# vinits5/bullet-envs

Hardware: AMD Instinct MI355X
Metric: env-steps/sec (whole node), 16-link snake, 4096 envs/GPU (higher is better)
Workload: dtype f32

## Files before the change

bullet-envs_amd/csrc/snk_dynamics.hpp:

```cpp
#pragma once
#include "snk_lds.hpp"
#include "snk_model.hpp"
#include "snk_wave.hpp"

namespace snk {

#ifndef SNK_SCALAR_DYNAMICS
__device__ __forceinline__ float quad_yzx(float x) {
    return __int_as_float(__builtin_amdgcn_update_dpp(0, __float_as_int(x), 0xC9, 0xf, 0xf, true));
}
__device__ __forceinline__ float quad_zxy(float x) {
    return __int_as_float(__builtin_amdgcn_update_dpp(0, __float_as_int(x), 0xD2, 0xf, 0xf, true));
}
__device__ __forceinline__ float lane_cross(float a_yzx, float a_zxy, float b) {
#pragma clang fp contract(off)
    return __builtin_fmaf(a_yzx, quad_zxy(b), -(a_zxy * quad_yzx(b)));
}
struct LaneVel {
    float w, v, za, zl;
};
__device__ __forceinline__ LaneVel lane_vel_step(float wp, float vp, float ax, float rb, float qdb) {
#pragma clang fp contract(off)
    const float wy = quad_yzx(wp), wz = quad_zxy(wp);
    const float cr = lane_cross(wy, wz, rb);
    LaneVel o;
    o.w = __builtin_fmaf(ax, qdb, wp);
    o.v = vp + cr;
    o.za = lane_cross(wy, wz, ax) * qdb;
    o.zl = lane_cross(wy, wz, cr);
    return o;
}
#endif

template <class LT>
__device__ void fk_vel(LT& L, const DevModel& M, int lane) {
    constexpr int N = LT::kN;
    const float* bs = L.base();
    float Rp[9];
    quat_rot(bs[3], bs[4], bs[5], bs[6], Rp);
    f3 op = ld3(bs), wp = ld3(bs + 7), vp = ld3(bs + 10);
    if (lane == 0) {
#pragma unroll
        for (int i = 0; i < 9; i++) L.R[0][i] = Rp[i];
        st3(L.o[0], op); st3(L.w[0], wp); st3(L.v[0], vp);
        st3(L.r[0], mk3(0, 0, 0)); st3(L.ax[0], mk3(0, 0, 0));
#pragma unroll
        for (int i = 0; i < 6; i++) L.zeta[0][i] = 0.f;
    }
    float snv = 0.f, csv = 1.f;
    if (lane < N) sincosf(L.q()[lane], &snv, &csv);
#ifndef SNK_SCALAR_DYNAMICS
    const int ln = launder_lane(lane);
    const int c = ln & 3, cc = c < 3 ? c : 2;
    float C0 = c == 0 ? Rp[0] : (c == 1 ? Rp[3] : Rp[6]);
    float C1 = c == 0 ? Rp[1] : (c == 1 ? Rp[4] : Rp[7]);
    float C2 = c == 0 ? Rp[2] : (c == 1 ? Rp[5] : Rp[8]);
    float opv = bs[cc], wpv = bs[7 + cc], vpv = bs[10 + cc];
#pragma unroll 4
    for (int b = 1; b <= N; b++) {
#pragma clang fp contract(off)
        const float* Rf = M.Rfix[b];
        const float* pf = M.pfix[b];
        const float qdb = L.qd()[b - 1];
        const float sn = __int_as_float(__builtin_amdgcn_readlane(__float_as_int(snv), b - 1));
        const float cs = __int_as_float(__builtin_amdgcn_readlane(__float_as_int(csv), b - 1));
        const float T0 = __builtin_fmaf(C2, Rf[6], __builtin_fmaf(C0, Rf[0], C1 * Rf[3]));
        const float T1 = __builtin_fmaf(C2, Rf[7], __builtin_fmaf(C0, Rf[1], C1 * Rf[4]));
        const float T2 = __builtin_fmaf(C2, Rf[8], __builtin_fmaf(C0, Rf[2], C1 * Rf[5]));
        const float N0 = __builtin_fmaf(T0, cs, -(sn * T2));
        const float N2 = __builtin_fmaf(sn, T0, cs * T2);
        const float rb = __builtin_fmaf(C2, pf[2], __builtin_fmaf(C0, pf[0], C1 * pf[1]));
        const float o = opv + rb;
        const LaneVel k = lane_vel_step(wpv, vpv, T1, rb, qdb);
        if (ln < 3) {
            L.R[b][3 * c] = N0; L.R[b][3 * c + 1] = T1; L.R[b][3 * c + 2] = N2;
            L.o[b][c] = o; L.r[b][c] = rb; L.ax[b][c] = T1; L.w[b][c] = k.w; L.v[b][c] = k.v;
            L.zeta[b][c] = k.za; L.zeta[b][3 + c] = k.zl;
        }
        C0 = N0; C1 = T1; C2 = N2;
        opv = o; wpv = k.w; vpv = k.v;
    }
#else
#pragma unroll 4
    for (int b = 1; b <= N; b++) {
        const float* Rf = M.Rfix[b];
        float T[9];
#pragma unroll
        for (int i = 0; i < 3; i++)
#pragma unroll
            for (int j = 0; j < 3; j++)
                T[3 * i + j] = Rp[3 * i] * Rf[j] + Rp[3 * i + 1] * Rf[3 + j] + Rp[3 * i + 2] * Rf[6 + j];
        float qdb = L.qd()[b - 1];
        const float sn = __int_as_float(__builtin_amdgcn_readlane(__float_as_int(snv), b - 1));
        const float cs = __int_as_float(__builtin_amdgcn_readlane(__float_as_int(csv), b - 1));
        float Rn[9];
#pragma unroll
        for (int i = 0; i < 3; i++) {
            Rn[3 * i + 0] = cs * T[3 * i] - sn * T[3 * i + 2];
            Rn[3 * i + 1] = T[3 * i + 1];
            Rn[3 * i + 2] = sn * T[3 * i] + cs * T[3 * i + 2];
        }
        f3 rb = mulRv(Rp, ld3(M.pfix[b]));
        f3 o = op + rb;
        f3 ax = mk3(T[1], T[4], T[7]);
        f3 w = wp + ax * qdb;
        f3 v = vp + cross(wp, rb);
        f3 za = cross(wp, ax) * qdb;
        f3 zl = cross(wp, cross(wp, rb));
        if (lane == 0) {
#pragma unroll
            for (int i = 0; i < 9; i++) L.R[b][i] = Rn[i];
            st3(L.o[b], o); st3(L.r[b], rb); st3(L.ax[b], ax); st3(L.w[b], w); st3(L.v[b], v);
            st3(&L.zeta[b][0], za); st3(&L.zeta[b][3], zl);
        }
#pragma unroll
        for (int i = 0; i < 9; i++) Rp[i] = Rn[i];
        op = o; wp = w; vp = v;
    }
#endif
    lds_sync();
}

template <class LT>
__device__ __forceinline__ void vel_refresh(LT& L, int lane) {
    constexpr int N = LT::kN;
#ifdef SNK_SCALAR_DYNAMICS
    f3 wp = ld3(L.base() + 7), vp = ld3(L.base() + 10);
    if (lane == 0) { st3(L.w[0], wp); st3(L.v[0], vp); }
    for (int b = 1; b <= N; b++) {
        f3 ax = ld3(L.ax[b]), rb = ld3(L.r[b]);
        float qdb = L.qd()[b - 1];
        f3 w = wp + ax * qdb, v = vp + cross(wp, rb);
        f3 za = cross(wp, ax) * qdb, zl = cross(wp, cross(wp, rb));
        if (lane == 0) { st3(L.w[b], w); st3(L.v[b], v); st3(&L.zeta[b][0], za); st3(&L.zeta[b][3], zl); }
        wp = w; vp = v;
    }
#else
    const int ln = launder_lane(lane);
    const int c = ln & 3, cc = c < 3 ? c : 2;
    float wpv = L.base()[7 + cc], vpv = L.base()[10 + cc];
    if (ln < 3) { L.w[0][c] = wpv; L.v[0][c] = vpv; }
    for (int b = 1; b <= N; b++) {
        const LaneVel k = lane_vel_step(wpv, vpv, L.ax[b][cc], L.r[b][cc], L.qd()[b - 1]);
        if (ln < 3) { L.w[b][c] = k.w; L.v[b][c] = k.v; L.zeta[b][c] = k.za; L.zeta[b][3 + c] = k.zl; }
        wpv = k.w; vpv = k.v;
    }
#endif
}

template <class LT>
__device__ float mean_height(LT& L, const DevModel& M, int lane) {
    constexpr int N = LT::kN;
    float z = 0.f;
    if (lane == 0) z = L.o[0][2] + L.R[0][6] * M.hbase[0] + L.R[0][7] * M.hbase[1] + L.R[0][8] * M.hbase[2];
    else if (lane <= N) z = L.o[lane][2];
    return wave_sum<64>(z) * (1.0f / (N + 1));
}

template <class LT, bool FIRST>
__device__ void body_bias(LT& L, const DevModel& M, int lane) {
    constexpr int N = LT::kN;
    if (lane <= N) {
        const int b = lane;
        const float* R = L.R[b];
        f3 w = ld3(L.w[b]), v = ld3(L.v[b]);
        float m = M.mass[b];
        f3 cw = mulRv(R, ld3(M.com[b]));
        float Ibar[6];
        rotSym(R, M.Ib[b], Ibar);
        f3 pN = cross(w, mulSv(Ibar, w));
        f3 pF = cross(w, cross(w, cw)) * m;
        float Irw[6];
        rotSym(R, M.Irot[b], Irw);
        float nw = sqrtf(dot(w, w));
        pN = pN + mulSv(Irw, w) * (M.ang_damp + M.ang_damp * nw);
        const int ns = M.nsub[b];
        for (int s = 0; s < ns; s++) {
            f3 cs = mulRv(R, ld3(M.sub_c[b][s]));
            f3 vs = v + cross(w, cs);
            float nv = sqrtf(dot(vs, vs));
            f3 F = vs * (M.sub_m[b][s] * (M.lin_damp + M.lin_damp * nv));
            pF = pF + F;
            pN = pN + cross(cs, F);
        }
        if (FIRST) {
            f3 G = mk3(0.f, 0.f, m * M.gz);
            pF = pF - G;
            pN = pN - cross(cw, G);
            st3(L.cw[b], cw);
            float* IA = L.IA[b];
#pragma unroll
            for (int i = 0; i < 6; i++) IA[i] = Ibar[i];
            float hx = m * cw.x, hy = m * cw.y, hz = m * cw.z;
            IA[6] = 0.f; IA[7] = -hz; IA[8] = hy;
            IA[9] = hz;  IA[10] = 0.f; IA[11] = -hx;
            IA[12] = -hy; IA[13] = hx; IA[14] = 0.f;
            IA[15] = m; IA[16] = 0.f; IA[17] = 0.f; IA[18] = m; IA[19] = 0.f; IA[20] = m;
        } else {
            pN = pN - ld3(L.ext(b));
            pF = pF - ld3(L.ext(b) + 3);
        }
        st3(&L.p[b][0], pN);
        st3(&L.p[b][3], pF);
    }
}

template <class LT, bool FACTOR>
__device__ void aba_main(LT& L, const DevModel& M, int lane SNK_PROF_F_PARAM) {
    constexpr int N = LT::kN;
    float cA[6], cB[9], cC[6];
#pragma unroll
    for (int i = 0; i < 6; i++) { cA[i] = 0.f; cC[i] = 0.f; }
#pragma unroll
    for (int i = 0; i < 9; i++) cB[i] = 0.f;
    f3 cN = mk3(0, 0, 0), cF = mk3(0, 0, 0);
    for (int b = N; b >= 1; b--) {
        float A[6], B[9], C[6];
        float* IA = L.IA[b];
#pragma unroll
        for (int i = 0; i < 6; i++) { A[i] = IA[i]; C[i] = IA[15 + i]; }
#pragma unroll
        for (int i = 0; i < 9; i++) B[i] = IA[6 + i];
        if (FACTOR) {
#pragma unroll
            for (int i = 0; i < 6; i++) { A[i] += cA[i]; C[i] += cC[i]; }
#pragma unroll
            for (int i = 0; i < 9; i++) B[i] += cB[i];
        }
        f3 pN = ld3(&L.p[b][0]) + cN, pF = ld3(&L.p[b][3]) + cF;
        f3 ax = ld3(L.ax[b]);
        f3 Ua, Ub;
        float Dinv;
        if (FACTOR) {
            Ua = mulSv(A, ax);
            Ub = mk3(B[0] * ax.x + B[3] * ax.y + B[6] * ax.z, B[1] * ax.x + B[4] * ax.y + B[7] * ax.z,
                     B[2] * ax.x + B[5] * ax.y + B[8] * ax.z);
            Dinv = 1.0f / dot(ax, Ua);
        } else {
            Ua = ld3(L.Ua[b]); Ub = ld3(L.Ub[b]); Dinv = L.Dinv[b];
        }
        f3 za = ld3(&L.zeta[b][0]), zl = ld3(&L.zeta[b][3]);
        float u = L.tauj[b - 1] - dot(ax, pN);
        f3 tN = mulSv(A, za) + mk3(B[0] * zl.x + B[1] * zl.y + B[2] * zl.z, B[3] * zl.x + B[4] * zl.y + B[5] * zl.z,
                                   B[6] * zl.x + B[7] * zl.y + B[8] * zl.z);
        f3 tF = mk3(B[0] * za.x + B[3] * za.y + B[6] * za.z, B[1] * za.x + B[4] * za.y + B[7] * za.z,
                    B[2] * za.x + B[5] * za.y + B[8] * za.z) + mulSv(C, zl);
        float uz = dot(Ua, za) + dot(Ub, zl);
        float s = (u - uz) * Dinv;
        f3 paN = pN + tN + Ua * s, paF = pF + tF + Ub * s;
        f3 r = ld3(L.r[b]);
        cN = paN + cross(r, paF);
        cF = paF;
        if (lane == 0) {
            L.u[b] = u;
            if (FACTOR) {
#pragma unroll
                for (int i = 0; i < 6; i++) { IA[i] = A[i]; IA[15 + i] = C[i]; }
#pragma unroll
                for (int i = 0; i < 9; i++) IA[6 + i] = B[i];
                st3(L.Ua[b], Ua); st3(L.Ub[b], Ub); L.Dinv[b] = Dinv;
            }
        }
        if (FACTOR) {
            float ua[3] = {Ua.x, Ua.y, Ua.z}, ub[3] = {Ub.x, Ub.y, Ub.z};
            float Ap[6], Bp[9], Cp[6];
            Ap[0] = A[0] - ua[0] * ua[0] * Dinv; Ap[1] = A[1] - ua[0] * ua[1] * Dinv; Ap[2] = A[2] - ua[0] * ua[2] * Dinv;
            Ap[3] = A[3] - ua[1] * ua[1] * Dinv; Ap[4] = A[4] - ua[1] * ua[2] * Dinv; Ap[5] = A[5] - ua[2] * ua[2] * Dinv;
            Cp[0] = C[0] - ub[0] * ub[0] * Dinv; Cp[1] = C[1] - ub[0] * ub[1] * Dinv; Cp[2] = C[2] - ub[0] * ub[2] * Dinv;
            Cp[3] = C[3] - ub[1] * ub[1] * Dinv; Cp[4] = C[4] - ub[1] * ub[2] * Dinv; Cp[5] = C[5] - ub[2] * ub[2] * Dinv;
#pragma unroll
            for (int i = 0; i < 3; i++)
#pragma unroll
                for (int j = 0; j < 3; j++) Bp[3 * i + j] = B[3 * i + j] - ua[i] * ub[j] * Dinv;
            f3 c0 = cross(r, mk3(Cp[0], Cp[1], Cp[2]));
            f3 c1 = cross(r, mk3(Cp[1], Cp[3], Cp[4]));
            f3 c2 = cross(r, mk3(Cp[2], Cp[4], Cp[5]));
            float Bn[9] = {Bp[0] + c0.x, Bp[1] + c1.x, Bp[2] + c2.x, Bp[3] + c0.y, Bp[4] + c1.y, Bp[5] + c2.y,
                           Bp[6] + c0.z, Bp[7] + c1.z, Bp[8] + c2.z};
            f3 e0 = cross(r, mk3(Bp[0], Bp[1], Bp[2])), e1 = cross(r, mk3(Bp[3], Bp[4], Bp[5])),
               e2 = cross(r, mk3(Bp[6], Bp[7], Bp[8]));
            f3 g0 = cross(r, mk3(Bn[0], Bn[1], Bn[2])), g1 = cross(r, mk3(Bn[3], Bn[4], Bn[5])),
               g2 = cross(r, mk3(Bn[6], Bn[7], Bn[8]));
            cA[0] = Ap[0] + e0.x + g0.x;
            cA[1] = Ap[1] + e0.y + g1.x;
            cA[2] = Ap[2] + e0.z + g2.x;
            cA[3] = Ap[3] + e1.y + g1.y;
            cA[4] = Ap[4] + e1.z + g2.y;
            cA[5] = Ap[5] + e2.z + g2.z;
#pragma unroll
            for (int i = 0; i < 9; i++) cB[i] = Bn[i];
#pragma unroll
            for (int i = 0; i < 6; i++) cC[i] = Cp[i];
        }
    }
    SNK_FSTAMP(2)
    f3 pN = ld3(&L.p[0][0]) + cN, pF = ld3(&L.p[0][3]) + cF;
    float p0[6] = {pN.x, pN.y, pN.z, pF.x, pF.y, pF.z};
    if (FACTOR) {
        float* IA = L.IA[0];
        float A[6], B[9], C[6];
#pragma unroll
        for (int i = 0; i < 6; i++) { A[i] = IA[i] + cA[i]; C[i] = IA[15 + i] + cC[i]; }
#pragma unroll
        for (int i = 0; i < 9; i++) B[i] = IA[6 + i] + cB[i];
        float G[6][6];
        G[0][0] = A[0]; G[0][1] = A[1]; G[0][2] = A[2]; G[1][1] = A[3]; G[1][2] = A[4]; G[2][2] = A[5];
        G[1][0] = A[1]; G[2][0] = A[2]; G[2][1] = A[4];
        G[3][3] = C[0]; G[3][4] = C[1]; G[3][5] = C[2]; G[4][4] = C[3]; G[4][5] = C[4]; G[5][5] = C[5];
        G[4][3] = C[1]; G[5][3] = C[2]; G[5][4] = C[4];
#pragma unroll
        for (int i = 0; i < 3; i++)
#pragma unroll
            for (int j = 0; j < 3; j++) { G[i][3 + j] = B[3 * i + j]; G[3 + j][i] = B[3 * i + j]; }
        float V[6][6];
#pragma unroll
        for (int i = 0; i < 6; i++)
#pragma unroll
            for (int j = 0; j < 6; j++) V[i][j] = (i == j) ? 1.f : 0.f;
#pragma unroll
        for (int k = 0; k < 6; k++) {
            float piv = 1.0f / G[k][k];
#pragma unroll
            for (int j = 0; j < 6; j++) { G[k][j] *= piv; V[k][j] *= piv; }
#pragma unroll
            for (int i = 0; i < 6; i++) {
                if (i != k) {
                    float f = G[i][k];
#pragma unroll
                    for (int j = 0; j < 6; j++) { G[i][j] -= f * G[k][j]; V[i][j] -= f * V[k][j]; }
                }
            }
        }
        if (lane == 0) {
#pragma unroll
            for (int i = 0; i < 6; i++)
#pragma unroll
                for (int j = 0; j < 6; j++) L.Inv0[6 * i + j] = V[i][j];
        }
        float a0[6];
#pragma unroll
        for (int i = 0; i < 6; i++) {
            float s = 0.f;
#pragma unroll
            for (int j = 0; j < 6; j++) s -= V[i][j] * p0[j];
            a0[i] = s;
        }
        if (lane == 0) {
#pragma unroll
            for (int i = 0; i < 6; i++) L.acc0[i] = a0[i];
        }
    } else {
        float a0[6];
#pragma unroll
        for (int i = 0; i < 6; i++) {
            float s = 0.f;
#pragma unroll
            for (int j = 0; j < 6; j++) s -= L.Inv0[6 * i + j] * p0[j];
            a0[i] = s;
        }
        if (lane == 0) {
#pragma unroll
            for (int i = 0; i < 6; i++) L.acc0[i] = a0[i];
        }
    }
    lds_sync();
    SNK_FSTAMP(3)
    if (!FACTOR) return;
    f3 al = ld3(&L.acc0[0]), a = ld3(&L.acc0[3]);
    for (int b = 1; b <= N; b++) {
        f3 r = ld3(L.r[b]);
        f3 ap = a + cross(al, r) + ld3(&L.zeta[b][3]);
        f3 alp = al + ld3(&L.zeta[b][0]);
        float qdd = (L.u[b] - (dot(ld3(L.Ua[b]), alp) + dot(ld3(L.Ub[b]), ap))) * L.Dinv[b];
        al = alp + ld3(L.ax[b]) * qdd;
        a = ap;
        if (lane == 0) L.qdd[b - 1] = qdd;
    }
    lds_sync();
    SNK_FSTAMP(4)
}

template <class LT>
__device__ __forceinline__ bool sensor_pass_needed(LT& L, const DevModel& M, int lane, float dv, const SensorHint& hint) {
    constexpr int N = LT::kN;
    constexpr int ND = N + 6;
    if (hint.always) return true;
    const float dt = M.dt;
    float e = 0.f, wgt = 0.f;
    if (lane < ND) {
        const float vold = lane < 6 ? L.base()[7 + lane] : L.qd()[lane - 6];
        const float x = fminf(fmaxf(vold + dv, -M.max_vel), M.max_vel);
        if (lane >= 6) e = L.targets[lane - 6] - (L.q()[lane - 6] + dt * x);
        const int m = N + 5 - lane;
        const float arm = lane < 3 ? (M.reach_hb + M.reach_l * (0.5f * N * (N + 1))) * (1.0f / (N + 1))
                                   : (lane < 6 ? 1.0f : M.reach_l * ((float)(m * (m + 1)) * (0.5f / (N + 1))));
        wgt = fabsf(x) * arm;
    }
    const float se = wave_sum<64>(e * e);
    const float reach = dt * wave_sum<64>(wgt) + kReachSlack;
    const float tol = M.servo_tol * 1.001f;
    const bool sensor = !(se > tol * tol) || hint.counter_next > M.max_counter || !(hint.h_prev + reach < M.height_thr);
    return __builtin_amdgcn_readfirstlane(sensor ? 1 : 0) != 0;
}

__device__ __forceinline__ void step_base_pose(float* bs, float dt, int lane) {
    f3 om = ld3(bs + 7), vl = ld3(bs + 10);
    float fA = sqrtf(dot(om, om));
    const float kThr = 0.78539816339744831f;
    if (fA * dt > kThr) fA = kThr / dt;
    float sc;
    if (fA < 0.001f) sc = 0.5f * dt - (dt * dt * dt) * 0.020833333333f * fA * fA;
    else sc = sinf(0.5f * fA * dt) / fA;
    float dx = om.x * sc, dy = om.y * sc, dz = om.z * sc, dw = cosf(fA * dt * 0.5f);
    float qx = bs[3], qy = bs[4], qz = bs[5], qw = bs[6];
    float nw = dw * qw - dx * qx - dy * qy - dz * qz;
    float nx = dw * qx + dx * qw + dy * qz - dz * qy;
    float ny = dw * qy - dx * qz + dy * qw + dz * qx;
    float nz = dw * qz + dx * qy - dy * qx + dz * qw;
    float inv = 1.0f / sqrtf(nx * nx + ny * ny + nz * nz + nw * nw);
    lds_sync();
    if (lane == 0) {
        bs[0] += dt * vl.x; bs[1] += dt * vl.y; bs[2] += dt * vl.z;
        bs[3] = nx * inv; bs[4] = ny * inv; bs[5] = nz * inv; bs[6] = nw * inv;
    }
}

}
```

Before: 380,800.

## Distribute ABA inward articulated-inertia recursion across lanes using DPP quad shuffles

Replaces the per-thread inward pass of the articulated-body algorithm (in the FACTOR path) with a lane-parallel version. Each lane owns a few entries of the 21-element spatial inertia and of the bias force. Cross products use DPP row shuffles, and U/D/p values are broadcast with readlane. The root inertia and bias are written to a new Inv0 buffer that the base solve reads. This cuts serial per-lane arithmetic and register pressure in the recursion, at the cost of many cross-lane operations, LDS stores and intricate index logic.

After: 380,700, median of 2. No clear change (-0.0%).

```diff
diff --git a/bullet-envs_amd/csrc/snk_dynamics.hpp b/bullet-envs_amd/csrc/snk_dynamics.hpp
--- a/bullet-envs_amd/csrc/snk_dynamics.hpp
+++ b/bullet-envs_amd/csrc/snk_dynamics.hpp
@@ -205,6 +205,106 @@
     }
 }
 
+#ifndef SNK_SCALAR_DYNAMICS
+__device__ __forceinline__ float up_yzx(float x) {
+    return __int_as_float(__builtin_amdgcn_update_dpp(0, __float_as_int(x), 0x108, 0xf, 0xf, true));
+}
+__device__ __forceinline__ float up_zxy(float x) {
+    return __int_as_float(__builtin_amdgcn_update_dpp(0, __float_as_int(x), 0x10C, 0xf, 0xf, true));
+}
+__device__ __forceinline__ float lane_cross_up(float r_yzx, float r_zxy, float f) {
+#pragma clang fp contract(off)
+    return __builtin_fmaf(r_yzx, up_zxy(f), -(r_zxy * up_yzx(f)));
+}
+typedef __attribute__((address_space(3))) float lds_float;
+__device__ __forceinline__ lds_float* lane_ptr(float* p) {
+    unsigned a = (unsigned)(size_t)(lds_float*)p;
+    asm volatile("" : "+v"(a));
+    return (lds_float*)(size_t)a;
+}
+template <class LT>
+__device__ __forceinline__ void aba_inward_lanes(LT& L, int lane) {
+#pragma clang fp contract(off)
+    constexpr int N = LT::kN;
+    const int ln = launder_lane(lane);
+    const int c = ln & 3, qd = (ln >> 2) & 3;
+    const int rot = (c < 3 ? c : 2) + (qd > 1 ? qd - 1 : 0), cc = rot < 3 ? rot : rot - 3;
+    const int bt = qd != 0;
+    const bool bot = bt != 0, own = ln < 7 && c < 3;
+    const int s1 = cc == 0 ? 1 : cc + 2, s2 = cc == 0 ? 2 : cc + 3;
+    const int o0 = bot ? 6 + cc : cc, o1 = bot ? 9 + cc : s1, o2 = bot ? 12 + cc : s2;
+    const int o3 = bot ? 15 + cc : 6 + 3 * cc, o4 = bot ? 15 + s1 : 7 + 3 * cc, o5 = bot ? 15 + s2 : 8 + 3 * cc;
+    const int v0 = (!bot && cc == 0) ? o0 : o5, v1 = (!bot && cc <= 1) ? o1 : o5, v2 = !bot ? o2 : o5;
+    const int v3 = (!bot || cc == 0) ? o3 : o5, v4 = (!bot || cc <= 1) ? o4 : o5;
+    const int pi = 3 * bt + cc;
+    const int c1 = cc == 2 ? 0 : cc + 1, c2 = cc == 0 ? 2 : cc - 1;
+    float* ia = &L.IA[0][0];
+    lds_float *l0 = lane_ptr(ia + o0), *l1 = lane_ptr(ia + o1), *l2 = lane_ptr(ia + o2), *l3 = lane_ptr(ia + o3),
+              *l4 = lane_ptr(ia + o4), *l5 = lane_ptr(ia + o5);
+    lds_float *t0 = lane_ptr(ia + v0), *t1 = lane_ptr(ia + v1), *t2 = lane_ptr(ia + v2), *t3 = lane_ptr(ia + v3),
+              *t4 = lane_ptr(ia + v4);
+    lds_float* lp = lane_ptr(&L.p[0][0] + pi);
+    lds_float *lry = lane_ptr(&L.r[0][0] + c1), *lrz = lane_ptr(&L.r[0][0] + c2);
+    lds_float* lu = lane_ptr(&L.Ua[0][0] + ((int)(&L.Ub[0][0] - &L.Ua[0][0]) * bt + cc));
+    float h0 = 0.f, h1 = 0.f, h2 = 0.f, h3 = 0.f, h4 = 0.f, h5 = 0.f, hp = 0.f;
+#pragma unroll 4
+    for (int b = N; b >= 1; b--) {
+        float x0 = l0[21 * b] + h0, x1 = l1[21 * b] + h1, x2 = l2[21 * b] + h2;
+        float x3 = l3[21 * b] + h3, x4 = l4[21 * b] + h4, x5 = l5[21 * b] + h5;
+        const float pv = lp[6 * b] + hp;
+        const f3 ax = ld3(L.ax[b]), za = ld3(&L.zeta[b][0]), zl = ld3(&L.zeta[b][3]), r = ld3(L.r[b]);
+        const float ry = lry[3 * b], rz = lrz[3 * b];
+        const float U = __builtin_fmaf(x2, ax.z, __builtin_fmaf(x0, ax.x, x1 * ax.y));
+        const float Ua0 = rdlane(U, 0), Ua1 = rdlane(U, 1), Ua2 = rdlane(U, 2);
+        const float Ub0 = rdlane(U, 4), Ub1 = rdlane(U, 5), Ub2 = rdlane(U, 6);
+        const float pN0 = rdlane(pv, 0), pN1 = rdlane(pv, 1), pN2 = rdlane(pv, 2);
+        const float D = __builtin_fmaf(ax.z, Ua2, __builtin_fmaf(ax.x, Ua0, ax.y * Ua1));
+        const float Dinv = 1.0f / D;
+        const float u = L.tauj[b - 1] - __builtin_fmaf(pN2, ax.z, __builtin_fmaf(pN0, ax.x, pN1 * ax.y));
+        const float t = __builtin_fmaf(x2, za.z, __builtin_fmaf(x0, za.x, x1 * za.y)) +
+                        __builtin_fmaf(x5, zl.z, __builtin_fmaf(x3, zl.x, x4 * zl.y));
+        const float uz = __builtin_fmaf(Ua2, za.z, __builtin_fmaf(Ua0, za.x, Ua1 * za.y)) +
+                         __builtin_fmaf(Ub2, zl.z, __builtin_fmaf(Ub0, zl.x, Ub1 * zl.y));
+        const float s = (u - uz) * Dinv;
+        const float pa = __builtin_fmaf(U, s, pv + t);
+        const float cr = lane_cross_up(ry, rz, pa);
+        hp = bot ? pa : pa + cr;
+        if (ln == 0) { L.u[b] = u; L.Dinv[b] = Dinv; }
+        if (own) {
+            lu[3 * b] = U;
+            t0[21 * b] = x0; t1[21 * b] = x1; t2[21 * b] = x2; t3[21 * b] = x3; t4[21 * b] = x4; l5[21 * b] = x5;
+        }
+        x0 = __builtin_fmaf(-(U * Ua0), Dinv, x0); x1 = __builtin_fmaf(-(U * Ua1), Dinv, x1);
+        x2 = __builtin_fmaf(-(U * Ua2), Dinv, x2); x3 = __builtin_fmaf(-(U * Ub0), Dinv, x3);
+        x4 = __builtin_fmaf(-(U * Ub1), Dinv, x4); x5 = __builtin_fmaf(-(U * Ub2), Dinv, x5);
+        const float k0 = __builtin_fmaf(r.y, x5, -(r.z * x4)), k1 = __builtin_fmaf(r.z, x3, -(r.x * x5)),
+                    k2 = __builtin_fmaf(r.x, x4, -(r.y * x3));
+        float k1o = __builtin_fmaf(-r.x, x5, r.z * x3);
+        asm volatile("" : "+v"(k1o));
+        const float k1b = cc == 1 ? k1o : k1;
+        const float y0 = x0 + k0, y1 = x1 + k1b, y2 = x2 + k2;
+        float m1o = __builtin_fmaf(-rz, up_yzx(x4), ry * up_zxy(x4)), m1s = lane_cross_up(ry, rz, x4);
+        asm volatile("" : "+v"(m1o), "+v"(m1s));
+        const float m1 = cc == 1 ? m1o : m1s;
+        const float n3 = x3 + lane_cross_up(ry, rz, x3), n4 = x4 + m1, n5 = x5 + lane_cross_up(ry, rz, x5);
+        const float g0 = __builtin_fmaf(r.y, n5, -(r.z * n4)), g1 = __builtin_fmaf(r.z, n3, -(r.x * n5));
+        const float e0 = lane_cross_up(ry, rz, x0), e1 = lane_cross_up(ry, rz, x1);
+        const float f1 = lane_cross_up(ry, rz, y1), f2 = lane_cross_up(ry, rz, y2);
+        const float a0 = (x0 + e0) + g0;
+        const float a1 = (x1 + (cc == 0 ? k1 : e1)) + (cc == 0 ? f1 : g1);
+        const float a2 = (x2 + k2) + f2;
+        h0 = bot ? y0 : a0; h1 = bot ? y1 : a1; h2 = bot ? y2 : a2;
+        h3 = bot ? x3 : n3; h4 = bot ? x4 : n4; h5 = bot ? x5 : n5;
+    }
+    const float x0 = l0[0] + h0, x1 = l1[0] + h1, x2 = l2[0] + h2, x3 = l3[0] + h3, x4 = l4[0] + h4, x5 = l5[0] + h5;
+    const float pv = lp[0] + hp;
+    if (own) {
+        float* st = L.Inv0;
+        st[v0] = x0; st[v1] = x1; st[v2] = x2; st[v3] = x3; st[v4] = x4; st[o5] = x5; st[21 + pi] = pv;
+    }
+}
+#endif
+
 template <class LT, bool FACTOR>
 __device__ void aba_main(LT& L, const DevModel& M, int lane SNK_PROF_F_PARAM) {
     constexpr int N = LT::kN;
@@ -214,6 +314,10 @@
 #pragma unroll
     for (int i = 0; i < 9; i++) cB[i] = 0.f;
     f3 cN = mk3(0, 0, 0), cF = mk3(0, 0, 0);
+#ifndef SNK_SCALAR_DYNAMICS
+    if (FACTOR) aba_inward_lanes(L, lane);
+    else
+#endif
     for (int b = N; b >= 1; b--) {
         float A[6], B[9], C[6];
         float* IA = L.IA[b];
@@ -295,14 +399,25 @@
     }
     SNK_FSTAMP(2)
     f3 pN = ld3(&L.p[0][0]) + cN, pF = ld3(&L.p[0][3]) + cF;
+#ifndef SNK_SCALAR_DYNAMICS
+    if (FACTOR) { pN = ld3(&L.Inv0[21]); pF = ld3(&L.Inv0[24]); }
+#endif
     float p0[6] = {pN.x, pN.y, pN.z, pF.x, pF.y, pF.z};
     if (FACTOR) {
+        float A[6], B[9], C[6];
+#ifndef SNK_SCALAR_DYNAMICS
+        const float* IA = L.Inv0;
+#pragma unroll
+        for (int i = 0; i < 6; i++) { A[i] = IA[i]; C[i] = IA[15 + i]; }
+#pragma unroll
+        for (int i = 0; i < 9; i++) B[i] = IA[6 + i];
+#else
         float* IA = L.IA[0];
-        float A[6], B[9], C[6];
 #pragma unroll
         for (int i = 0; i < 6; i++) { A[i] = IA[i] + cA[i]; C[i] = IA[15 + i] + cC[i]; }
 #pragma unroll
         for (int i = 0; i < 9; i++) B[i] = IA[6 + i] + cB[i];
+#endif
         float G[6][6];
         G[0][0] = A[0]; G[0][1] = A[1]; G[0][2] = A[2]; G[1][1] = A[3]; G[1][2] = A[4]; G[2][2] = A[5];
         G[1][0] = A[1]; G[2][0] = A[2]; G[2][1] = A[4];
```
